# qurAI-amsterdam/SuperResolution_aniso_MRI

Hardware: AMD Instinct MI355X
Metric: training slices/sec (ae_combined, 160x160, latent=128) (higher is better)
Workload: dtype f32; 1 GPU; ACDC synthetic 12x(3x1x160x160) triplets, ae_combined latent=128 depth=32 scales=2, MSE synthesis loss (BASELINE configs[1]); global_batch_triplets=12, parallelism=dp1, init=reference Initializer, seed 892372, random weights, launch=captured HIP graph replay

## Files before the change

superresolution_aniso_mri_amd/csrc/aesr_api.hip:

```cpp
#include <stdarg.h>
#include <stdio.h>
#include <stdlib.h>
#include <string.h>

#include <map>
#include <mutex>
#include <tuple>

#include "../../include/aesr_hip.h"
#include "../../include/aesr_hip_dataprep.h"
#include "aesr_kernels.h"

static thread_local char g_err[512] = "";
void aesr_set_error(const char* fmt, ...) {
    va_list ap;
    va_start(ap, fmt);
    vsnprintf(g_err, sizeof(g_err), fmt, ap);
    va_end(ap);
}

static void cout_padding(int Cout, int* CoutP, int* NB) {
    if (Cout <= 16) { *CoutP = 16; *NB = 1; }
    else if (Cout <= 32) { *CoutP = 32; *NB = 2; }
    else { *CoutP = round_up(Cout, 64); *NB = 4; }
// ... 675 lines not shown
    a.dy = dy; a.w = w; a.dx = dx; a.N = N; a.H = H; a.W = W; a.Cin = Cin; a.Cout = Cout; a.KS = KS; a.pad = pad; a.bcast = bcast;
    a.Ho = H + 2 * pad - KS + 1; a.Wo = W + 2 * pad - KS + 1;
    for (int i = 0; i < Cin && bcast; ++i) a.ca[i] = ca_host[i];
    return aesr_launch_smallcin_dgrad(a, (hipStream_t)stream);
}

#define SMALL_WGRAD_NWG 512
size_t aesr_small_wgrad_workspace_floats(int nout) { return (size_t)SMALL_WGRAD_NWG * nout; }

int aesr_conv2d_smallcin_wgrad(const float* in, const float* dout, float* dw, float* db, float* workspace, int N, int H,
                               int W, int Cin, int Cout, int pad, void* stream) {
    AESR_CHECK_ARG(in && dout && dw && db && workspace && Cin >= 1 && Cin <= 4, "aesr_conv2d_smallcin_wgrad: need 1 <= Cin <= 4");
    AESR_CHECK_ARG(Cout >= 4 && Cout % 4 == 0 && 256 % (Cout / 4) == 0 && Cout <= 256,
                   "aesr_conv2d_smallcin_wgrad: Cout=%d must be a multiple of 4 with Cout/4 dividing 256", Cout);
    SmallWgradArgs a;
    a.in = in; a.dout = dout; a.partial = workspace; a.N = N; a.H = H; a.W = W; a.Cin = Cin; a.Cout = Cout; a.pad = pad;
    a.Ho = H + 2 * pad; a.Wo = W + 2 * pad;
    if (int e = aesr_launch_smallcin_wgrad(a, SMALL_WGRAD_NWG, (hipStream_t)stream)) return e;
    return aesr_launch_sum_partials(workspace, SMALL_WGRAD_NWG, Cout * (Cin + 1), dw, Cout * Cin, db, (hipStream_t)stream);
}

int aesr_conv2d_cout1_fwd(const float* x, const float* w, const float* bias, float* out, int N, int H, int W, int Cin, int act,
                          float slope, void* stream) {
    AESR_CHECK_ARG(x && w && out && N > 0 && H > 0 && W > 0, "aesr_conv2d_cout1_fwd: null pointer or empty shape");
    AESR_CHECK_ARG(Cin > 0 && Cin % 4 == 0 && Cin <= 256, "aesr_conv2d_cout1_fwd: Cin=%d must be a multiple of 4 (<= 256)", Cin);
    if (((Cin / 4) & (Cin / 4 - 1)) == 0)
        return aesr_launch_thin_collapse(x, w, bias, out, N, H, W, Cin, act, slope, (hipStream_t)stream);
    Cout1FwdArgs a;
    a.x = x; a.w = w; a.bias = bias; a.out = out; a.N = N; a.H = H; a.W = W; a.Cin = Cin; a.act = act; a.slope = slope;
    a.TH = H < 16 ? H : 16; a.TW = W < 16 ? W : 16;
    while (((size_t)(a.TH + 2) * (a.TW + 2) * (Cin + 4) + 9 * Cin) * 4 > 64 * 1024 && a.TH > 1) a.TH /= 2;
    a.tiles_y = ceil_div(H, a.TH); a.tiles_x = ceil_div(W, a.TW);
    return aesr_launch_cout1_fwd(a, (hipStream_t)stream);
}

#define THIN_NWG 512
static bool thin_channels_ok(int C) { return C >= 4 && C <= 256 && C % 4 == 0 && ((C / 4) & (C / 4 - 1)) == 0; }

size_t aesr_conv2d_cout1_workspace_floats(int Cin) {
    const size_t legacy = (size_t)SMALL_WGRAD_NWG * (Cin * 9 + 1);
    const size_t thin = (size_t)(THIN_NWG + 1) * 10 * Cin;
    return legacy > thin ? legacy : thin;
}

int aesr_conv2d_cout1_wgrad(const float* x, const float* dy, float* dw, float* db, float* workspace, int N, int H, int W,
                            int Cin, void* stream) {
    AESR_CHECK_ARG(x && dy && dw && db && workspace, "aesr_conv2d_cout1_wgrad: null pointer");
    AESR_CHECK_ARG(N > 0 && H > 0 && W > 0, "aesr_conv2d_cout1_wgrad: empty shape");
    if (thin_channels_ok(Cin)) {
        ThinArgs a;
        memset(&a, 0, sizeof(a));
        a.s = dy; a.t = x; a.partial = workspace;
        a.N = N; a.Hs = H; a.Ws = W; a.Ho = H; a.Wo = W; a.C = Cin; a.ps = 0; a.with_be = 0;
        float* R = workspace + (size_t)THIN_NWG * 10 * Cin;
        if (int e = aesr_launch_thin_reduce(a, THIN_NWG, (hipStream_t)stream)) return e;
        if (int e = aesr_launch_sum_partials(workspace, THIN_NWG, 10 * Cin, R, 10 * Cin, nullptr, (hipStream_t)stream)) return e;
        return aesr_launch_thin_cout1_finish(R, dw, db, Cin, (hipStream_t)stream);
    }
    AESR_CHECK_ARG(Cin >= 4 && Cin <= 128 && 256 % Cin == 0, "aesr_conv2d_cout1_wgrad: Cin=%d must divide 256 (and be >= 4)", Cin);
    Cout1WgradArgs a;
    a.x = x; a.dy = dy; a.partial = workspace; a.N = N; a.H = H; a.W = W; a.Cin = Cin;
    a.TH = H < 16 ? H : 16; a.TW = W < 16 ? W : 16;
    while ((size_t)(a.TH + 2) * (a.TW + 2) * (Cin + 1) * 4 > 60 * 1024 && a.TH > 1) a.TH /= 2;
    a.tiles_y = ceil_div(H, a.TH); a.tiles_x = ceil_div(W, a.TW); a.ntiles = N * a.tiles_y * a.tiles_x;
    int nwg = a.ntiles < SMALL_WGRAD_NWG ? a.ntiles : SMALL_WGRAD_NWG;
    if (int e = aesr_launch_cout1_wgrad(a, nwg, (hipStream_t)stream)) return e;
    return aesr_launch_sum_partials(workspace, nwg, Cin * 9 + 1, dw, Cin * 9, db, (hipStream_t)stream);
}

int aesr_conv2d_cout1_dgrad(const float* dy, const float* w, const float* y_saved, float* dx, float* workspace, int N, int H,
                            int W, int Cin, int mask_act, float slope, void* stream) {
    AESR_CHECK_ARG(dy && w && dx && workspace && N > 0 && H > 0 && W > 0, "aesr_conv2d_cout1_dgrad: null pointer or empty shape");
    AESR_CHECK_ARG(thin_channels_ok(Cin), "aesr_conv2d_cout1_dgrad: Cin=%d must be 4 times a power of two (4..256)", Cin);
    if (int e = aesr_launch_thin_cout1_flip(w, workspace, Cin, (hipStream_t)stream)) return e;
    ThinArgs a;
    memset(&a, 0, sizeof(a));
    a.s = dy; a.w = workspace; a.ysave = y_saved; a.out = dx;
    a.N = N; a.Hs = H; a.Ws = W; a.Ho = H; a.Wo = W; a.C = Cin; a.ps = 0;
    a.act = ACT_NONE; a.mask_act = y_saved ? mask_act : ACT_NONE; a.slope = slope;
    return aesr_launch_thin_expand(a, (hipStream_t)stream);
}

int aesr_conv2d_cout1_dgrad_pre(const float* dy, const float* w_flipped, const float* y_saved, float* dx, int N, int H, int W, int Cin,
                                int mask_act, float slope, void* stream) {
    AESR_CHECK_ARG(dy && w_flipped && dx && N > 0 && H > 0 && W > 0, "aesr_conv2d_cout1_dgrad_pre: null pointer or empty shape");
    AESR_CHECK_ARG(thin_channels_ok(Cin), "aesr_conv2d_cout1_dgrad_pre: Cin=%d must be 4 times a power of two (4..256)", Cin);
    ThinArgs a;
    memset(&a, 0, sizeof(a));
    a.s = dy; a.w = w_flipped; a.ysave = y_saved; a.out = dx;
    a.N = N; a.Hs = H; a.Ws = W; a.Ho = H; a.Wo = W; a.C = Cin; a.ps = 0;
    a.act = ACT_NONE; a.mask_act = y_saved ? mask_act : ACT_NONE; a.slope = slope;
    return aesr_launch_thin_expand(a, (hipStream_t)stream);
}

size_t aesr_stemconv_folded_floats(int C1) { return (size_t)2 * 9 * C1; }

int aesr_stemconv_fold(const float* w_stem, const float* b_stem, const float* w1, float* folded, int Cs, int C1, void* stream) {
    AESR_CHECK_ARG(w_stem && w1 && folded && Cs > 0 && C1 > 0, "aesr_stemconv_fold: bad arguments");
    return aesr_launch_thin_stem_fold(w_stem, b_stem, w1, folded, Cs, C1, (hipStream_t)stream);
}

int aesr_stemconv_fwd(const float* x, const float* folded, const float* b1, float* out, int N, int H, int W, int C1,
                      int stem_pad, int act, float slope, void* stream) {
    AESR_CHECK_ARG(x && folded && out && N > 0 && H > 0 && W > 0 && stem_pad >= 0, "aesr_stemconv_fwd: bad arguments");
    AESR_CHECK_ARG(thin_channels_ok(C1), "aesr_stemconv_fwd: C1=%d must be 4 times a power of two (4..256)", C1);
    ThinArgs a;
    memset(&a, 0, sizeof(a));
    a.s = x; a.w = folded; a.be = folded + (size_t)9 * C1; a.b = b1; a.out = out;
    a.N = N; a.Hs = H; a.Ws = W; a.Ho = H + 2 * stem_pad; a.Wo = W + 2 * stem_pad; a.C = C1; a.ps = stem_pad;
    a.act = act; a.mask_act = ACT_NONE; a.slope = slope;
// ... 469 lines not shown
```

superresolution_aniso_mri_amd/csrc/aesr_kernels.h:

```cpp
#pragma once
#include "aesr_common.h"

struct IgemmArgs {
    const float* in; const float* wpk; const float* bias; const float* ysave; float* out;
    int N, H, W, Cin, CinP, Cout, CoutP, Ho, Wo, pad;
    int TI, TH, TW, tiles_y, tiles_x, nitems, dbg;
    int NT;
    int ksplit;
    float* dbgbuf;
    int act, mask_act;
    float slope;
};
int aesr_launch_conv_igemm(const IgemmArgs& a, int KS, int NB, int MBW, hipStream_t st);
int aesr_launch_conv_ksplit_fixup(const float* partial, const float* bias, const float* ysave, float* out, size_t nelem, int Cout,
                                  int ksplit, int act, int mask_act, float slope, hipStream_t st);
int aesr_launch_pack_weights(const float* w, float* p, int Cout, int Cin, int KS, int KinP, int NoutP, int TN, int transpose, hipStream_t st);

struct WinoArgs {
    const float* in; const float* upk; const float* bias; const float* ysave; float* out;
    int N, H, W, Cin, CinP, Cout, CoutP;
    int TI, THt, TWt;
    int regs_y, regs_x, nitems;
    unsigned m_ncot, m_regs_x, m_regs_y;
    int act, mask_act;
// ... 60 lines not shown
    int act, mask_act;
    float slope;
    int transpose, bcast;
    float ca[4], cb[4];
};
struct SmallDgradArgs {
    const float* dy; const float* w; float* dx;
    int N, H, W, Cin, Cout, Ho, Wo, KS, pad, bcast;
    float ca[4];
};
struct SmallWgradArgs {
    const float* in; const float* dout; float* partial;
    int N, H, W, Cin, Cout, Ho, Wo, pad;
};
struct Cout1WgradArgs {
    const float* x; const float* dy; float* partial;
    int N, H, W, Cin, TH, TW, tiles_y, tiles_x, ntiles;
};
struct Cout1FwdArgs {
    const float* x; const float* w; const float* bias; float* out;
    int N, H, W, Cin, TH, TW, tiles_y, tiles_x, act;
    float slope;
};
int aesr_launch_cout1_fwd(const Cout1FwdArgs& a, hipStream_t st);
int aesr_launch_smallcin_fwd(const SmallArgs& a, hipStream_t st);
int aesr_launch_smallcin_dgrad(const SmallDgradArgs& a, hipStream_t st);
int aesr_launch_sum_partials(const float* partial, int np, int n, float* out0, int n0, float* out1, hipStream_t st);
int aesr_launch_smallcin_wgrad(const SmallWgradArgs& a, int nwg, hipStream_t st);
int aesr_launch_cout1_wgrad(const Cout1WgradArgs& a, int nwg, hipStream_t st);

struct ThinArgs {
    const float* s;
    const float* w;
    const float* be;
    const float* b;
    const float* ysave;
    float* out;
    const float* t;
    float* partial;
    int N, Hs, Ws, Ho, Wo, C, ps;
    int act, mask_act;
    float slope;
    int with_be;
    int tiles_y, tiles_x, ntiles;
};
int aesr_launch_thin_expand(ThinArgs a, hipStream_t st);
int aesr_launch_thin_reduce(ThinArgs a, int nwg, hipStream_t st);
int aesr_launch_thin_collapse(const float* x, const float* w, const float* bias, float* out, int N, int H, int W, int C, int act,
                              float slope, hipStream_t st);
int aesr_launch_thin_stem_fold(const float* ws, const float* bs, const float* w1, float* folded, int Cs, int C1, hipStream_t st);
int aesr_launch_thin_stem_finish(const float* R, const float* ws, const float* bs, const float* w1, float* dws, float* dbs,
                                 float* dw1, float* db1, int Cs, int C1, hipStream_t st);
int aesr_launch_thin_cout1_flip(const float* w, float* wexp, int Cin, hipStream_t st);
int aesr_launch_thin_cout1_finish(const float* R, float* dw, float* db, int Cin, hipStream_t st);

struct BnGroups { int G; int nstart[5]; };
struct BnApplyArgs {
    const float* y; const float* scale; const float* shift; float* out;
    int N, H, W, C, Ho, Wo, mode;
    BnGroups gr;
};
struct BnBwdArgs {
    const float* gout; const float* y; const float* mean; const float* invstd; const float* scale; const float* coef;
    float* partial; float* dpre;
    int N, H, W, C, Ho, Wo, mode, act;
    float slope;
    BnGroups gr;
    unsigned long long m_hw, m_w;
    int k_hw, k_w;
};
struct BnFusedArgs;
struct BnP2P { int world, rank, slot; const unsigned* gen; void* peers[8]; };
int aesr_launch_p2p_tick(unsigned* gen, hipStream_t st);
bool aesr_bn_fused1_ok(int N, int H, int W, int C, int pool, int G, int backward);
unsigned aesr_bn_fused_timeouts_impl();
int aesr_bn_fused_run(const float* y, const float* gout, float* out, float* rec, unsigned* bar, const float* gamma, const float* beta,
                      float* running_mean, float* running_var, long long* nbt, float* mean, float* invstd, float* scale, float* shift, float* coef,
                      float* dgamma, float* dbeta, int N, int H, int W, int C, int pool, int G, const int* nstart, const double* counts,
                      float momentum, float eps, int update_running, int act, float slope, int backward, const BnP2P* p2p, hipStream_t st);
int aesr_launch_bn_stats(const float* y, float* partial, int HW, int C, const BnGroups& gr, int nwg, hipStream_t st);
int aesr_launch_bn_reduce(const float* partial, double* sums, int nwg, int C, int G, hipStream_t st);
int aesr_launch_bn_finalize(const double* sums, const double* counts, const float* gamma, const float* beta, float* rm, float* rv,
                            long long* nbt, float* mean, float* invstd, float* scale, float* shift, int C, int G, float momentum,
                            float eps, int train, int update_running, hipStream_t st);
int aesr_launch_bn_reduce_finalize(const float* partial, int nwg, const double* counts, const float* gamma, const float* beta,
                                   float* running_mean, float* running_var, long long* nbt, float* mean, float* invstd,
                                   float* scale, float* shift, int C, int G, float momentum, float eps, int update_running,
                                   hipStream_t st);
int aesr_launch_bn_bwd_reduce_finalize(const float* partial, int nwg, const double* counts, float* coef, float* dgamma,
                                       float* dbeta, int C, int G, hipStream_t st);
int aesr_launch_bn_apply(const BnApplyArgs& a, hipStream_t st);
int aesr_launch_bn_bwd_reduce(const BnBwdArgs& a, int nwg, hipStream_t st);
int aesr_launch_bn_bwd_finalize(const double* sums, const double* counts, float* coef, float* dgamma, float* dbeta, int C, int G, hipStream_t st);
int aesr_launch_bn_bwd_apply(const BnBwdArgs& a, hipStream_t st);
bool aesr_bn_fused_ok(int C, int G);
int aesr_launch_bn_finalize_apply(const double* sums, const double* counts, const float* gamma, const float* beta, float* running_mean,
                                  float* running_var, long long* nbt, float* mean, float* invstd, float* scale, float* shift, float momentum,
                                  float eps, int update_running, int G, const BnApplyArgs& a, hipStream_t st);
int aesr_launch_bn_bwd_finalize_apply(const double* sums, const double* counts, float* coef, float* dgamma, float* dbeta, int G,
                                      const BnBwdArgs& a, hipStream_t st);

int aesr_launch_lerp_fwd(const float* z, const float* af, const float* at, float* zmix, int B, size_t per, hipStream_t st);
int aesr_launch_lerp_bwd(const float* dmix, const float* af, const float* at, float* dz, int B, size_t per, hipStream_t st);
int aesr_launch_lerp_cat_fwd(const float* z, const float* af, const float* at, float* zcat, int B, size_t per, hipStream_t st);
int aesr_launch_interleave_clamp(const float* orig, const float* synth, float* out, int Z, int n, size_t per, float lo, float hi, hipStream_t st);
int aesr_launch_lerp_multi(const float* z, float* out, int Z, size_t per, const float* alphas, int n, float nslope, hipStream_t st);
int aesr_launch_lerp_cat_bwd(const float* g, const float* af, const float* at, float* dz, int B, size_t per, hipStream_t st);
// ... 40 lines not shown
```

superresolution_aniso_mri_amd/csrc/conv_thin.hip:

```cpp
#include "aesr_kernels.h"
#include "aesr_pack_dev.h"

#define THIN_TH 8
#ifndef THIN_ETH
#define THIN_ETH 16
#endif
#define THIN_XS 68

__host__ __device__ __forceinline__ int thin_tw(int C4) { return 256 / C4 < 64 ? 256 / C4 : 64; }

template <int TH = THIN_TH>
__device__ __forceinline__ void thin_stage(const ThinArgs& a, float (*xs)[THIN_XS], int n, int y0, int x0, int TW) {
    const int PW = TW + 2;
    for (int q = threadIdx.x; q < (TH + 2) * PW; q += 256) {
        const int r = q / PW, c = q - r * PW;
        const int sy = y0 + r - 1 - a.ps, sx = x0 + c - 1 - a.ps;
        float v = 0.f;
        if (sy >= 0 && sy < a.Hs && sx >= 0 && sx < a.Ws) v = a.s[((size_t)n * a.Hs + sy) * a.Ws + sx];
        xs[r][c] = v;
    }
}

__global__ __launch_bounds__(256) void thin_expand_kernel(ThinArgs a) {
    __shared__ float xs[THIN_ETH + 2][THIN_XS];
// ... 54 lines not shown
            for (int e = 0; e < 4; ++e) acc[e] *= act_grad_from_output(ys[e], a.mask_act, a.slope);
        }
        *(f32x4*)(a.out + o) = acc;
    }
}

template <bool WITH_BE>
__global__ __launch_bounds__(256) void thin_reduce_kernel(ThinArgs a) {
    __shared__ float xs[THIN_TH + 2][THIN_XS];
    extern __shared__ __attribute__((aligned(16))) float red[];
    constexpr int NROW = WITH_BE ? 19 : 10;
    const int C4 = a.C >> 2, TW = thin_tw(C4);
    const int tid = threadIdx.x, c4 = tid % C4, pl = tid / C4;
    const int lane = tid & 63, wave = tid >> 6;
    f32x4 accW[9], accB[9];
    float accs = 0.f;
#pragma unroll
    for (int t = 0; t < 9; ++t) {
        accW[t] = (f32x4){0.f, 0.f, 0.f, 0.f};
        accB[t] = (f32x4){0.f, 0.f, 0.f, 0.f};
    }
    const int tpi = a.tiles_y * a.tiles_x;
    for (int tile = blockIdx.x; tile < a.ntiles; tile += gridDim.x) {
        const int n = tile / tpi;
        const int trem = tile - n * tpi;
        const int ty = trem / a.tiles_x, tx = trem - ty * a.tiles_x;
        const int y0 = ty * THIN_TH, x0 = tx * TW;
        __syncthreads();
        thin_stage(a, xs, n, y0, x0, TW);
        const int ox = x0 + pl;
        const bool xin = pl < TW && ox < a.Wo;
        const int plr = pl < TW ? pl : 0;
        f32x4 g[THIN_TH];
#pragma unroll
        for (int r = 0; r < THIN_TH; ++r) {
            const int oy = y0 + r;
            g[r] = (f32x4){0.f, 0.f, 0.f, 0.f};
            if (xin && oy < a.Ho) g[r] = *(const f32x4*)(a.t + (((size_t)n * a.Ho + oy) * a.Wo + ox) * a.C + c4 * 4);
        }
        float mxf[3];
        mxf[0] = (ox - 1 >= 0) ? 1.f : 0.f;
        mxf[1] = 1.f;
        mxf[2] = (ox + 1 < a.Wo) ? 1.f : 0.f;
        __syncthreads();
#pragma unroll
        for (int r = 0; r < THIN_TH; ++r) {
            const int oy = y0 + r;
#pragma unroll
            for (int t = 0; t < 9; ++t) {
                const float v = xs[r + t / 3][plr + t % 3];
#pragma unroll
                for (int e = 0; e < 4; ++e) accW[t][e] = fmaf(g[r][e], v, accW[t][e]);
            }
            if (WITH_BE) {
#pragma unroll
                for (int dy = 0; dy < 3; ++dy) {
                    const int yy = oy + dy - 1;
                    const float myf = (yy >= 0 && yy < a.Ho) ? 1.f : 0.f;
#pragma unroll
                    for (int dx = 0; dx < 3; ++dx) {
                        const float m = myf * mxf[dx];
#pragma unroll
                        for (int e = 0; e < 4; ++e) accB[dy * 3 + dx][e] = fmaf(g[r][e], m, accB[dy * 3 + dx][e]);
                    }
                }
            }
            if (c4 == 0 && xin && oy < a.Ho) accs += xs[r + 1][plr + 1];
        }
    }
    for (int m = C4; m < 64; m <<= 1) {
#pragma unroll
        for (int t = 0; t < 9; ++t)
#pragma unroll
            for (int e = 0; e < 4; ++e) {
                accW[t][e] += __shfl_xor(accW[t][e], m, 64);
                if (WITH_BE) accB[t][e] += __shfl_xor(accB[t][e], m, 64);
            }
    }
    for (int m = 1; m < 64; m <<= 1) accs += __shfl_xor(accs, m, 64);
    __syncthreads();
    if (lane < C4) {
        float* rw = red + (size_t)wave * NROW * a.C;
#pragma unroll
        for (int t = 0; t < 9; ++t) {
            *(f32x4*)(rw + t * a.C + c4 * 4) = accW[t];
            if (WITH_BE) *(f32x4*)(rw + (9 + t) * a.C + c4 * 4) = accB[t];
        }
        *(f32x4*)(rw + (NROW - 1) * a.C + c4 * 4) = (f32x4){c4 == 0 ? accs : 0.f, 0.f, 0.f, 0.f};
    }
    __syncthreads();
    const int nout = NROW * a.C;
    for (int o = tid; o < nout; o += 256)
        a.partial[(size_t)blockIdx.x * nout + o] =
            (red[o] + red[(size_t)nout + o]) + (red[2 * (size_t)nout + o] + red[3 * (size_t)nout + o]);
}

__global__ __launch_bounds__(256) void thin_collapse_kernel(const float* __restrict__ x, const float* __restrict__ w,
                                                            const float* __restrict__ bias, float* __restrict__ out, int N, int H,
                                                            int W, int C, int TH, int tiles_y, int tiles_x, int act, float slope) {
    __shared__ float S[2][3][4][64];
    const int C4 = C >> 2, TW = thin_tw(C4), TO = TW - 2;
    const int tid = threadIdx.x, c4 = tid % C4, pl = tid / C4;
    int tile = blockIdx.x;
    const int tx = tile % tiles_x;
    tile /= tiles_x;
    const int ty = tile % tiles_y;
    const int n = tile / tiles_y;
    const int y0 = ty * TH, x0 = tx * TO;
    const int xc = x0 - 1 + pl;
    const bool live = pl < TW && xc >= 0 && xc < W;
    f32x4 wq[9];
#pragma unroll
    for (int t = 0; t < 9; ++t)
#pragma unroll
        for (int e = 0; e < 4; ++e) wq[t][e] = w[(c4 * 4 + e) * 9 + t];
    const float b0 = bias ? bias[0] : 0.f;
    const f32x4 zero = {0.f, 0.f, 0.f, 0.f};
    const float* base = x + ((size_t)n * H * W + (live ? xc : 0)) * C + c4 * 4;
    auto load1 = [&](int yy) -> f32x4 {
        const f32x4 v = *(const f32x4*)(base + (size_t)min(max(yy, 0), H - 1) * W * C);
// ... 47 lines not shown


__global__ __launch_bounds__(256) void thin_stem_fold_kernel(const float* __restrict__ ws, const float* __restrict__ bs,
                                                             const float* __restrict__ w1, float* __restrict__ folded, int Cs,
                                                             int C1) {
    stem_fold_elements(ws, bs, w1, folded, Cs, C1, blockIdx.x * 256 + threadIdx.x, gridDim.x * 256);
}

__global__ __launch_bounds__(256) void thin_stem_finish_kernel(const float* __restrict__ R, const float* __restrict__ ws,
                                                               const float* __restrict__ bs, const float* __restrict__ w1,
                                                               float* __restrict__ dws, float* __restrict__ dbs,
                                                               float* __restrict__ dw1, float* __restrict__ db1, int Cs, int C1) {
    __shared__ double redw[256], redb[256];
    if ((int)blockIdx.x < Cs) {
        const int c = blockIdx.x;
        double sw = 0.0, sb = 0.0;
        for (int o = threadIdx.x; o < C1 * 9; o += 256) {
            const int co = o / 9, t = o - co * 9;
            const double wv = (double)w1[((size_t)co * Cs + c) * 9 + t];
            sw += wv * (double)R[t * C1 + co];
            sb += wv * (double)R[(9 + t) * C1 + co];
        }
        redw[threadIdx.x] = sw;
        redb[threadIdx.x] = sb;
        __syncthreads();
        for (int h = 128; h > 0; h >>= 1) {
            if ((int)threadIdx.x < h) {
                redw[threadIdx.x] += redw[threadIdx.x + h];
                redb[threadIdx.x] += redb[threadIdx.x + h];
            }
            __syncthreads();
        }
        if (threadIdx.x == 0) {
            dws[c] = (float)redw[0];
            if (dbs) dbs[c] = (float)redb[0];
        }
        return;
    }
    const int tid = (blockIdx.x - Cs) * 256 + threadIdx.x, nth = (gridDim.x - Cs) * 256;
    for (int o = tid; o < C1 * Cs * 9; o += nth) {
        const int t = o % 9, c = (o / 9) % Cs, co = o / (9 * Cs);
        float v = R[t * C1 + co] * ws[c];
        if (bs) v = fmaf(R[(9 + t) * C1 + co], bs[c], v);
        dw1[o] = v;
    }
    if (db1)
        for (int co = tid; co < C1; co += nth) db1[co] = R[(9 + 4) * C1 + co];
}

__global__ __launch_bounds__(256) void thin_cout1_flip_kernel(const float* __restrict__ w, float* __restrict__ wexp, int Cin) {
    cout1_flip_elements(w, wexp, Cin, blockIdx.x * 256 + threadIdx.x, gridDim.x * 256);
}

__global__ __launch_bounds__(256) void thin_cout1_finish_kernel(const float* __restrict__ R, float* __restrict__ dw,
                                                                float* __restrict__ db, int Cin) {
    for (int o = blockIdx.x * 256 + threadIdx.x; o < 9 * Cin; o += gridDim.x * 256) {
        const int ci = o / 9, k = o - ci * 9;
        dw[o] = R[(8 - k) * Cin + ci];
    }
    if (db && blockIdx.x == 0 && threadIdx.x == 0) db[0] = R[9 * Cin];
}


static bool thin_shape_ok(const ThinArgs& a) {
    const int C4 = a.C / 4;
    return a.C >= 4 && a.C % 4 == 0 && a.C <= 256 && (C4 & (C4 - 1)) == 0;
}

int aesr_launch_thin_expand(ThinArgs a, hipStream_t st) {
    if (!thin_shape_ok(a)) {
        aesr_set_error("thin conv: C=%d must be 4 times a power of two (4..256)", a.C);
        return AESR_ERR_ARG;
    }
    const int TW = thin_tw(a.C / 4);
    a.tiles_y = ceil_div(a.Ho, THIN_ETH);
    a.tiles_x = ceil_div(a.Wo, TW);
    a.ntiles = a.N * a.tiles_y * a.tiles_x;
    hipLaunchKernelGGL(thin_expand_kernel, dim3(a.ntiles), dim3(256), 0, st, a);
    AESR_LAUNCH_CHECK("thin_expand");
    return AESR_OK;
}

int aesr_launch_thin_reduce(ThinArgs a, int nwg, hipStream_t st) {
    if (!thin_shape_ok(a)) {
        aesr_set_error("thin conv: C=%d must be 4 times a power of two (4..256)", a.C);
        return AESR_ERR_ARG;
    }
    const int TW = thin_tw(a.C / 4);
    a.tiles_y = ceil_div(a.Ho, THIN_TH);
    a.tiles_x = ceil_div(a.Wo, TW);
    a.ntiles = a.N * a.tiles_y * a.tiles_x;
    const int nrow = a.with_be ? 19 : 10;
    const size_t shmem = (size_t)4 * nrow * a.C * sizeof(float);
    if (a.with_be)
        hipLaunchKernelGGL(thin_reduce_kernel<true>, dim3(nwg), dim3(256), shmem, st, a);
    else
        hipLaunchKernelGGL(thin_reduce_kernel<false>, dim3(nwg), dim3(256), shmem, st, a);
    AESR_LAUNCH_CHECK("thin_reduce");
    return AESR_OK;
}

int aesr_launch_thin_collapse(const float* x, const float* w, const float* bias, float* out, int N, int H, int W, int C, int act,
                              float slope, hipStream_t st) {
    const int C4 = C / 4;
    if (C < 4 || C % 4 != 0 || C > 256 || (C4 & (C4 - 1)) != 0) {
        aesr_set_error("thin conv: C=%d must be 4 times a power of two (4..256)", C);
        return AESR_ERR_ARG;
    }
    const int TW = thin_tw(C4), TH = H < 20 ? H : 20;
    const int tiles_y = ceil_div(H, TH), tiles_x = ceil_div(W, TW - 2);
    hipLaunchKernelGGL(thin_collapse_kernel, dim3(N * tiles_y * tiles_x), dim3(256), 0, st, x, w, bias, out, N, H, W, C, TH, tiles_y,
                       tiles_x, act, slope);
    AESR_LAUNCH_CHECK("thin_collapse");
    return AESR_OK;
}

int aesr_launch_thin_stem_fold(const float* ws, const float* bs, const float* w1, float* folded, int Cs, int C1, hipStream_t st) {
    hipLaunchKernelGGL(thin_stem_fold_kernel, dim3(ceil_div(9 * C1, 256)), dim3(256), 0, st, ws, bs, w1, folded, Cs, C1);
    AESR_LAUNCH_CHECK("thin_stem_fold");
    return AESR_OK;
}

int aesr_launch_thin_stem_finish(const float* R, const float* ws, const float* bs, const float* w1, float* dws, float* dbs,
                                 float* dw1, float* db1, int Cs, int C1, hipStream_t st) {
    int grid = ceil_div(C1 * Cs * 9, 256);
    if (grid > 64) grid = 64;
    hipLaunchKernelGGL(thin_stem_finish_kernel, dim3(Cs + grid), dim3(256), 0, st, R, ws, bs, w1, dws, dbs, dw1, db1, Cs, C1);
    AESR_LAUNCH_CHECK("thin_stem_finish");
    return AESR_OK;
}

int aesr_launch_thin_cout1_flip(const float* w, float* wexp, int Cin, hipStream_t st) {
    hipLaunchKernelGGL(thin_cout1_flip_kernel, dim3(ceil_div(9 * Cin, 256)), dim3(256), 0, st, w, wexp, Cin);
    AESR_LAUNCH_CHECK("thin_cout1_flip");
    return AESR_OK;
}

int aesr_launch_thin_cout1_finish(const float* R, float* dw, float* db, int Cin, hipStream_t st) {
    hipLaunchKernelGGL(thin_cout1_finish_kernel, dim3(ceil_div(9 * Cin, 256)), dim3(256), 0, st, R, dw, db, Cin);
    AESR_LAUNCH_CHECK("thin_cout1_finish");
    return AESR_OK;
}
```

superresolution_aniso_mri_amd/csrc/conv_wgrad_wino.hip:

```cpp
#include <stdio.h>
#include <stdlib.h>

#include <type_traits>
#include <utility>

#include "aesr_kernels.h"

constexpr int WW_OOB = 0x70000000;
typedef float f32x2 __attribute__((ext_vector_type(2)));
#ifndef WW_ABL
#define WW_ABL 0
#endif

template <int... I, class F>
__device__ __forceinline__ void ww_for(std::integer_sequence<int, I...>, F&& f) {
    (f(std::integral_constant<int, I>{}), ...);
}
template <int N, class F>
__device__ __forceinline__ void ww_rep(F&& f) { ww_for(std::make_integer_sequence<int, N>{}, f); }

__device__ __forceinline__ void ww_dma(__amdgpu_buffer_rsrc_t rs, float* lds_wave_base, int byte_off) {
    __builtin_amdgcn_raw_ptr_buffer_load_lds(rs, (__attribute__((address_space(3))) void*)lds_wave_base, 16, byte_off, 0, 0, 0);
}

// ... 130 lines not shown
            constexpr int i = decltype(Kc)::value >> 2, c = decltype(Kc)::value & 3;
            const unsigned ad = lx[i][c] + (unsigned)(xu * 4);
            f32x2 &p0_ = P[i][c][0], &p1_ = P[i][c][1];
            asm volatile("ds_read2st64_b32 %0, %2 offset0:%3 offset1:%4\n\tds_read2st64_b32 %1, %2 offset0:%5 offset1:%6"
                         : "=&v"(p0_), "=&v"(p1_) : "v"(ad), "n"(0), "n"(PWL / 2), "n"(PWL), "n"(3 * PWL / 2) : "memory");
        });
        ww_rep<4>([&](auto Kc) {
            constexpr int o = decltype(Kc)::value >> 1, e = decltype(Kc)::value & 1;
            const unsigned ad = ld[o][e] + (unsigned)(du * 4);
            f32x2& y_ = Mp[nb][o][e];
            asm volatile("ds_read2st64_b32 %0, %1 offset0:0 offset1:%2" : "=&v"(y_) : "v"(ad), "n"(TWL / 2) : "memory");
        });
    };
    auto op_transform = [&](int nb) {
        asm volatile("s_waitcnt lgkmcnt(0)" ::: "memory");
        ww_rep<2>([&](auto Ic) {
            constexpr int i = decltype(Ic)::value;
            f32x2 T[2][4];
            ww_rep<4>([&](auto Cc) {
                constexpr int c = decltype(Cc)::value;
                WW_PK(T[0][c], P[i][c][0], P[i][c][1], WW_M_T01);
                WW_PK(T[1][c], P[i][c][0], P[i][c][1], WW_M_T23);
            });
            ww_rep<2>([&](auto Sc) {
                constexpr int s_ = decltype(Sc)::value;
                WW_PK(Vp[nb][i][s_][0], T[s_][0], T[s_][2], WW_M_SUB);
                WW_PK(Vp[nb][i][s_][1], T[s_][1], T[s_][2], WW_M_ADD);
                WW_PK(Vp[nb][i][s_][2], T[s_][2], T[s_][1], WW_M_SUB);
                WW_PK(Vp[nb][i][s_][3], T[s_][1], T[s_][3], WW_M_SUB);
            });
        });
        ww_rep<2>([&](auto Oc) {
            constexpr int o = decltype(Oc)::value;
            WW_PK(Mp[nb][o][2], Mp[nb][o][0], Mp[nb][o][0], WW_M_SELF);
            WW_PK(Mp[nb][o][3], Mp[nb][o][1], Mp[nb][o][1], WW_M_SELF);
            WW_PK(Mp[nb][o][4], Mp[nb][o][0], Mp[nb][o][1], WW_M_LL);
            WW_PK(Mp[nb][o][7], Mp[nb][o][0], Mp[nb][o][1], WW_M_HH);
            WW_PK(Mp[nb][o][5], Mp[nb][o][2], Mp[nb][o][3], WW_M_LL);
            WW_PK(Mp[nb][o][6], Mp[nb][o][2], Mp[nb][o][3], WW_M_HH);
            accb[o] += Mp[nb][o][5][0];
        });
    };
    auto mfmas = [&](auto Q0c, auto Nc, int cb) {
        ww_rep<decltype(Nc)::value>([&](auto Dc) {
            constexpr int q = decltype(Q0c)::value + decltype(Dc)::value, x = q >> 2, i = (q >> 1) & 1, o = q & 1;
            constexpr int r = x >> 2, k = x & 3;
            constexpr int mi = k == 0 ? (r == 0 || r == 3 ? 0 : 2) : k == 3 ? (r == 0 || r == 3 ? 1 : 3) : 4 + r;
            constexpr int mh = k == 0 || k == 3 ? (r >= 2 ? 1 : 0) : k - 1;
            f32x4& acc_ = acc[x][i][o];
            const float va_ = Vp[cb][i][r >> 1][k][r & 1], vb_ = Mp[cb][o][mi][mh];
            asm volatile("v_mfma_f32_16x16x4_f32 %0, %1, %2, %0" : "+a"(acc_) : "v"(va_), "v"(vb_));
        });
    };
    auto step_xu = [&](int j, int buf) { const int ks = wave + 4 * j, tyl = ks / KPR, kx = ks - tyl * KPR; return buf * XFL + ((2 * tyl) * PWL + 8 * kx) * 32; };
    auto step_du = [&](int j, int buf) { const int ks = wave + 4 * j, tyl = ks / KPR, kx = ks - tyl * KPR; return buf * DFL + ((2 * tyl) * TWL + 8 * kx) * 32; };
    using C0 = std::integral_constant<int, 0>;
    using C16 = std::integral_constant<int, 16>;
    using C32 = std::integral_constant<int, 32>;

    long long tph[3] = {0, 0, 0}, tq = 0;
#define WW_STAMP(k)                                                   \
    if constexpr (STAMP) {                                            \
        const long long t_ = (long long)__builtin_amdgcn_s_memtime(); \
        tph[k] += t_ - tq;                                            \
        tq = t_;                                                      \
    }
    if constexpr (STAMP) tq = (long long)__builtin_amdgcn_s_memtime();

    WwTile t0, t1, t2;
    {
        t0.n = split / tpi;
        const int rem = split - t0.n * tpi;
        t0.ty = rem / a.tiles_x;
        t0.tx = rem - t0.ty * a.tiles_x;
        if (split >= a.ntiles) t0.n = a.N;
    }
    t1 = advance(t0);
    t2 = advance(t1);
    fetch(t0, 0);
    fetch(t1, 1);
    asm volatile("s_waitcnt vmcnt(0)" ::: "memory");
    __syncthreads();
    int buf = 0;
    op_read(step_xu(0, 0), step_du(0, 0), 0);
    op_transform(0);
    WW_STAMP(2)
    if (t0.n < a.N) do {
        __builtin_amdgcn_sched_barrier(0);
#if WW_ABL != 3 && WW_ABL != 4
        op_read(step_xu(1, buf), step_du(1, buf), 1);
#endif
        mfmas(C0{}, C16{}, 0);
#if WW_ABL != 2 && WW_ABL != 4
        op_transform(1);
#endif
        mfmas(C16{}, std::integral_constant<int, 48>{}, 0);
        __builtin_amdgcn_sched_barrier(0);
        WW_STAMP(0)
        asm volatile("s_waitcnt vmcnt(0) lgkmcnt(0)" ::: "memory");
        __syncthreads();
        WW_STAMP(1)
        __builtin_amdgcn_sched_barrier(0);
#if WW_ABL != 3 && WW_ABL != 4
        op_read(step_xu(0, buf ^ 1), step_du(0, buf ^ 1), 0);
#endif
        mfmas(C0{}, C16{}, 1);
        __builtin_amdgcn_sched_barrier(0);
#if WW_ABL != 1 && WW_ABL != 4
        fetch(t2, buf);
#endif
        __builtin_amdgcn_sched_barrier(0);
        mfmas(C16{}, C16{}, 1);
#if WW_ABL != 2 && WW_ABL != 4
        op_transform(0);
#endif
        mfmas(C32{}, C32{}, 1);
        __builtin_amdgcn_sched_barrier(0);
        t0 = t1;
        t1 = t2;
        t2 = advance(t2);
        buf ^= 1;
    } while (t0.n < a.N);
    WW_STAMP(0)
    asm volatile("s_waitcnt vmcnt(0) lgkmcnt(0)" ::: "memory");
    __syncthreads();
    if (STAMP && lane == 0)
        for (int k = 0; k < 3; ++k) a.dbgbuf[(blockIdx.x * 4 + wave) * 3 + k] = (float)tph[k];

    f32x4 dg[9][2][2];
#pragma unroll
    for (int i = 0; i < 2; ++i)
#pragma unroll
        for (int o = 0; o < 2; ++o) {
            f32x4 R[3][4];
#pragma unroll
            for (int j = 0; j < 4; ++j) {
                const f32x4 u0_ = acc[0 + j][i][o], u1 = acc[4 + j][i][o], u2 = acc[8 + j][i][o], u3 = -acc[12 + j][i][o];
                const f32x4 s = j == 3 ? (f32x4){-1.f, -1.f, -1.f, -1.f} : (f32x4){1.f, 1.f, 1.f, 1.f};
                R[0][j] = s * (u0_ + 0.5f * (u1 + u2));
                R[1][j] = s * (0.5f * (u1 - u2));
                R[2][j] = s * (0.5f * (u1 + u2) + u3);
            }
#pragma unroll
            for (int r = 0; r < 3; ++r) {
                dg[r * 3 + 0][i][o] = R[r][0] + 0.5f * (R[r][1] + R[r][2]);
                dg[r * 3 + 1][i][o] = 0.5f * (R[r][1] - R[r][2]);
                dg[r * 3 + 2][i][o] = 0.5f * (R[r][1] + R[r][2]) + R[r][3];
            }
        }
#pragma unroll
    for (int o = 0; o < 2; ++o) {
        accb[o] += __shfl_xor(accb[o], 16, 64);
        accb[o] += __shfl_xor(accb[o], 32, 64);
    }
    f32x4* ex = (f32x4*)lds;
    float* exb = lds + 4 * 36 * 64 * 4;
#pragma unroll
    for (int t = 0; t < 9; ++t)
#pragma unroll
        for (int i = 0; i < 2; ++i)
#pragma unroll
            for (int o = 0; o < 2; ++o) ex[(wave * 36 + (t * 4 + i * 2 + o)) * 64 + lane] = dg[t][i][o];
    if (g == 0) {
        exb[wave * 32 + l15] = accb[0];
        exb[wave * 32 + 16 + l15] = accb[1];
    }
    __syncthreads();
    const size_t plane = (size_t)a.CinP * a.CoutP;
    float* sl = a.slab + (size_t)split * 10 * plane;
// ... 95 lines not shown
```

Measured before the change: 15970 slices/s.

## Fuse thin cout1 partial sum into finish, hoist bias-grad sums, skip dead wgrad tiles

The thin Cout=1 weight-gradient path no longer runs a separate sum_partials launch. The finish kernel now reduces the per-workgroup partials directly, in double precision across 1024 threads, and scatters the result into dw/db. The thin reduce kernel builds bias-energy accumulators from per-tile row sums instead of per-row masked FMAs, which cuts inner-loop work. The Winograd wgrad kernel skips the second half-tile's LDS read, transform and MFMA groups when that half lies past the image bottom, using a scalar branch inside inline asm. This adds control-flow complexity and depends on the boundary logic being correct.

```diff
diff --git a/superresolution_aniso_mri_amd/csrc/aesr_api.hip b/superresolution_aniso_mri_amd/csrc/aesr_api.hip
--- a/superresolution_aniso_mri_amd/csrc/aesr_api.hip
+++ b/superresolution_aniso_mri_amd/csrc/aesr_api.hip
@@ -751,10 +751,8 @@
         memset(&a, 0, sizeof(a));
         a.s = dy; a.t = x; a.partial = workspace;
         a.N = N; a.Hs = H; a.Ws = W; a.Ho = H; a.Wo = W; a.C = Cin; a.ps = 0; a.with_be = 0;
-        float* R = workspace + (size_t)THIN_NWG * 10 * Cin;
         if (int e = aesr_launch_thin_reduce(a, THIN_NWG, (hipStream_t)stream)) return e;
-        if (int e = aesr_launch_sum_partials(workspace, THIN_NWG, 10 * Cin, R, 10 * Cin, nullptr, (hipStream_t)stream)) return e;
-        return aesr_launch_thin_cout1_finish(R, dw, db, Cin, (hipStream_t)stream);
+        return aesr_launch_thin_cout1_finish(workspace, THIN_NWG, dw, db, Cin, (hipStream_t)stream);
     }
     AESR_CHECK_ARG(Cin >= 4 && Cin <= 128 && 256 % Cin == 0, "aesr_conv2d_cout1_wgrad: Cin=%d must divide 256 (and be >= 4)", Cin);
     Cout1WgradArgs a;
diff --git a/superresolution_aniso_mri_amd/csrc/aesr_kernels.h b/superresolution_aniso_mri_amd/csrc/aesr_kernels.h
--- a/superresolution_aniso_mri_amd/csrc/aesr_kernels.h
+++ b/superresolution_aniso_mri_amd/csrc/aesr_kernels.h
@@ -136,7 +136,7 @@
 int aesr_launch_thin_stem_finish(const float* R, const float* ws, const float* bs, const float* w1, float* dws, float* dbs,
                                  float* dw1, float* db1, int Cs, int C1, hipStream_t st);
 int aesr_launch_thin_cout1_flip(const float* w, float* wexp, int Cin, hipStream_t st);
-int aesr_launch_thin_cout1_finish(const float* R, float* dw, float* db, int Cin, hipStream_t st);
+int aesr_launch_thin_cout1_finish(const float* partial, int np, float* dw, float* db, int Cin, hipStream_t st);
 
 struct BnGroups { int G; int nstart[5]; };
 struct BnApplyArgs {
diff --git a/superresolution_aniso_mri_amd/csrc/conv_thin.hip b/superresolution_aniso_mri_amd/csrc/conv_thin.hip
--- a/superresolution_aniso_mri_amd/csrc/conv_thin.hip
+++ b/superresolution_aniso_mri_amd/csrc/conv_thin.hip
@@ -130,20 +130,28 @@
 #pragma unroll
                 for (int e = 0; e < 4; ++e) accW[t][e] = fmaf(g[r][e], v, accW[t][e]);
             }
-            if (WITH_BE) {
-#pragma unroll
-                for (int dy = 0; dy < 3; ++dy) {
-                    const int yy = oy + dy - 1;
-                    const float myf = (yy >= 0 && yy < a.Ho) ? 1.f : 0.f;
-#pragma unroll
-                    for (int dx = 0; dx < 3; ++dx) {
-                        const float m = myf * mxf[dx];
-#pragma unroll
-                        for (int e = 0; e < 4; ++e) accB[dy * 3 + dx][e] = fmaf(g[r][e], m, accB[dy * 3 + dx][e]);
-                    }
-                }
-            }
             if (c4 == 0 && xin && oy < a.Ho) accs += xs[r + 1][plr + 1];
+        }
+        if (WITH_BE) {
+            f32x4 rest = g[1];
+#pragma unroll
+            for (int r = 2; r < THIN_TH; ++r) rest += g[r];
+            f32x4 sy[3];
+            sy[1] = rest + g[0];
+            sy[0] = y0 == 0 ? rest : sy[1];
+            sy[2] = sy[1];
+            if (y0 + THIN_TH >= a.Ho) {
+                sy[2] = (f32x4){0.f, 0.f, 0.f, 0.f};
+#pragma unroll
+                for (int r = 0; r < THIN_TH - 1; ++r)
+                    if (y0 + r < a.Ho - 1) sy[2] += g[r];
+            }
+#pragma unroll
+            for (int dy = 0; dy < 3; ++dy)
+#pragma unroll
+                for (int dx = 0; dx < 3; ++dx)
+#pragma unroll
+                    for (int e = 0; e < 4; ++e) accB[dy * 3 + dx][e] = fmaf(sy[dy][e], mxf[dx], accB[dy * 3 + dx][e]);
         }
     }
     for (int m = C4; m < 64; m <<= 1) {
@@ -297,13 +305,40 @@
     cout1_flip_elements(w, wexp, Cin, blockIdx.x * 256 + threadIdx.x, gridDim.x * 256);
 }
 
-__global__ __launch_bounds__(256) void thin_cout1_finish_kernel(const float* __restrict__ R, float* __restrict__ dw,
-                                                                float* __restrict__ db, int Cin) {
-    for (int o = blockIdx.x * 256 + threadIdx.x; o < 9 * Cin; o += gridDim.x * 256) {
-        const int ci = o / 9, k = o - ci * 9;
-        dw[o] = R[(8 - k) * Cin + ci];
-    }
-    if (db && blockIdx.x == 0 && threadIdx.x == 0) db[0] = R[9 * Cin];
+__global__ __launch_bounds__(1024) void thin_cout1_finish_kernel(const float* __restrict__ partial, int np, float* __restrict__ dw,
+                                                                 float* __restrict__ db, int Cin) {
+    __shared__ double red[16][64];
+    const int col = threadIdx.x & 63, rl = threadIdx.x >> 6;
+    const int o = blockIdx.x * 64 + col;
+    const int n = 10 * Cin, nuse = 9 * Cin + 1;
+    double s = 0.0;
+    if (o < nuse) {
+        double s0 = 0.0, s1 = 0.0, s2 = 0.0, s3 = 0.0;
+        int p = rl;
+        for (; p + 48 < np; p += 64) {
+            const float v0 = partial[(size_t)p * n + o], v1 = partial[(size_t)(p + 16) * n + o];
+            const float v2 = partial[(size_t)(p + 32) * n + o], v3 = partial[(size_t)(p + 48) * n + o];
+            s0 += (double)v0;
+            s1 += (double)v1;
+            s2 += (double)v2;
+            s3 += (double)v3;
+        }
+        for (; p < np; p += 16) s0 += (double)partial[(size_t)p * n + o];
+        s = (s0 + s1) + (s2 + s3);
+    }
+    red[rl][col] = s;
+    __syncthreads();
+    if (rl == 0 && o < nuse) {
+        s = 0.0;
+#pragma unroll
+        for (int k = 0; k < 16; ++k) s += red[k][col];
+        if (o < 9 * Cin) {
+            const int row = o / Cin, ci = o - row * Cin;
+            dw[ci * 9 + (8 - row)] = (float)s;
+        } else if (db) {
+            db[0] = (float)s;
+        }
+    }
 }
 
 
@@ -381,8 +416,8 @@
     return AESR_OK;
 }
 
-int aesr_launch_thin_cout1_finish(const float* R, float* dw, float* db, int Cin, hipStream_t st) {
-    hipLaunchKernelGGL(thin_cout1_finish_kernel, dim3(ceil_div(9 * Cin, 256)), dim3(256), 0, st, R, dw, db, Cin);
+int aesr_launch_thin_cout1_finish(const float* partial, int np, float* dw, float* db, int Cin, hipStream_t st) {
+    hipLaunchKernelGGL(thin_cout1_finish_kernel, dim3(ceil_div(9 * Cin + 1, 64)), dim3(1024), 0, st, partial, np, dw, db, Cin);
     AESR_LAUNCH_CHECK("thin_cout1_finish");
     return AESR_OK;
 }
diff --git a/superresolution_aniso_mri_amd/csrc/conv_wgrad_wino.hip b/superresolution_aniso_mri_amd/csrc/conv_wgrad_wino.hip
--- a/superresolution_aniso_mri_amd/csrc/conv_wgrad_wino.hip
+++ b/superresolution_aniso_mri_amd/csrc/conv_wgrad_wino.hip
@@ -206,6 +206,38 @@
             asm volatile("v_mfma_f32_16x16x4_f32 %0, %1, %2, %0" : "+a"(acc_) : "v"(va_), "v"(vb_));
         });
     };
+    auto mfmas_unless = [&](auto Q0c, auto Nc, int cb, int live) {
+        static_assert(decltype(Q0c)::value % 8 == 0 && decltype(Nc)::value % 8 == 0, "whole groups: positions x, x + 1 with all (i, o)");
+        ww_rep<decltype(Nc)::value / 8>([&](auto Gc) {
+            constexpr int x0 = (decltype(Q0c)::value >> 2) + 2 * decltype(Gc)::value, x1 = x0 + 1;
+            constexpr int r0 = x0 >> 2, k0 = x0 & 3, r1 = x1 >> 2, k1 = x1 & 3;
+            constexpr int mi0 = k0 == 0 ? (r0 == 0 || r0 == 3 ? 0 : 2) : k0 == 3 ? (r0 == 0 || r0 == 3 ? 1 : 3) : 4 + r0;
+            constexpr int mh0 = k0 == 0 || k0 == 3 ? (r0 >= 2 ? 1 : 0) : k0 - 1;
+            constexpr int mi1 = k1 == 0 ? (r1 == 0 || r1 == 3 ? 0 : 2) : k1 == 3 ? (r1 == 0 || r1 == 3 ? 1 : 3) : 4 + r1;
+            constexpr int mh1 = k1 == 0 || k1 == 3 ? (r1 >= 2 ? 1 : 0) : k1 - 1;
+            f32x4 &a0_ = acc[x0][0][0], &a1_ = acc[x0][0][1], &a2_ = acc[x0][1][0], &a3_ = acc[x0][1][1];
+            f32x4 &a4_ = acc[x1][0][0], &a5_ = acc[x1][0][1], &a6_ = acc[x1][1][0], &a7_ = acc[x1][1][1];
+            const float va00_ = Vp[cb][0][r0 >> 1][k0][r0 & 1], va01_ = Vp[cb][1][r0 >> 1][k0][r0 & 1];
+            const float va10_ = Vp[cb][0][r1 >> 1][k1][r1 & 1], va11_ = Vp[cb][1][r1 >> 1][k1][r1 & 1];
+            const float vb00_ = Mp[cb][0][mi0][mh0], vb01_ = Mp[cb][1][mi0][mh0];
+            const float vb10_ = Mp[cb][0][mi1][mh1], vb11_ = Mp[cb][1][mi1][mh1];
+            const int live_ = live;
+            asm volatile("s_cmp_lt_i32 %16, 1\n\t"
+                         "s_cbranch_scc1 .Lww_dead_%=\n\t"
+                         "v_mfma_f32_16x16x4_f32 %0, %8, %12, %0\n\t"
+                         "v_mfma_f32_16x16x4_f32 %1, %8, %13, %1\n\t"
+                         "v_mfma_f32_16x16x4_f32 %2, %9, %12, %2\n\t"
+                         "v_mfma_f32_16x16x4_f32 %3, %9, %13, %3\n\t"
+                         "v_mfma_f32_16x16x4_f32 %4, %10, %14, %4\n\t"
+                         "v_mfma_f32_16x16x4_f32 %5, %10, %15, %5\n\t"
+                         "v_mfma_f32_16x16x4_f32 %6, %11, %14, %6\n\t"
+                         "v_mfma_f32_16x16x4_f32 %7, %11, %15, %7\n"
+                         ".Lww_dead_%=:"
+                         : "+a"(a0_), "+a"(a1_), "+a"(a2_), "+a"(a3_), "+a"(a4_), "+a"(a5_), "+a"(a6_), "+a"(a7_)
+                         : "v"(va00_), "v"(va01_), "v"(va10_), "v"(va11_), "v"(vb00_), "v"(vb01_), "v"(vb10_), "v"(vb11_), "s"(live_)
+                         : "scc");
+        });
+    };
     auto step_xu = [&](int j, int buf) { const int ks = wave + 4 * j, tyl = ks / KPR, kx = ks - tyl * KPR; return buf * XFL + ((2 * tyl) * PWL + 8 * kx) * 32; };
     auto step_du = [&](int j, int buf) { const int ks = wave + 4 * j, tyl = ks / KPR, kx = ks - tyl * KPR; return buf * DFL + ((2 * tyl) * TWL + 8 * kx) * 32; };
     using C0 = std::integral_constant<int, 0>;
@@ -240,13 +272,15 @@
     op_transform(0);
     WW_STAMP(2)
     if (t0.n < a.N) do {
+        const int rows2 = __builtin_amdgcn_readfirstlane(a.H - (t0.ty * TH + TH / 2));
+        const bool dead = rows2 <= 0;
         __builtin_amdgcn_sched_barrier(0);
 #if WW_ABL != 3 && WW_ABL != 4
-        op_read(step_xu(1, buf), step_du(1, buf), 1);
+        if (!dead) op_read(step_xu(1, buf), step_du(1, buf), 1);
 #endif
         mfmas(C0{}, C16{}, 0);
 #if WW_ABL != 2 && WW_ABL != 4
-        op_transform(1);
+        if (!dead) op_transform(1);
 #endif
         mfmas(C16{}, std::integral_constant<int, 48>{}, 0);
         __builtin_amdgcn_sched_barrier(0);
@@ -258,17 +292,17 @@
 #if WW_ABL != 3 && WW_ABL != 4
         op_read(step_xu(0, buf ^ 1), step_du(0, buf ^ 1), 0);
 #endif
-        mfmas(C0{}, C16{}, 1);
+        mfmas_unless(C0{}, C16{}, 1, rows2);
         __builtin_amdgcn_sched_barrier(0);
 #if WW_ABL != 1 && WW_ABL != 4
         fetch(t2, buf);
 #endif
         __builtin_amdgcn_sched_barrier(0);
-        mfmas(C16{}, C16{}, 1);
+        mfmas_unless(C16{}, C16{}, 1, rows2);
 #if WW_ABL != 2 && WW_ABL != 4
         op_transform(0);
 #endif
-        mfmas(C32{}, C32{}, 1);
+        mfmas_unless(C32{}, C32{}, 1, rows2);
         __builtin_amdgcn_sched_barrier(0);
         t0 = t1;
         t1 = t2;
```

Result: no change. 16100 slices/s, median of 6 (+0.8%).
